# joaotavora/raytracing-one-weekend

Hardware: AMD Instinct MI355X
Metric: Msamples/sec (W×H×spp) on cover scene; achieved HBM GB/s vs peak (higher is better)
Workload: dtype f64

## Files before the change

### raytracing-one-weekend_amd/csrc/rtow_capi.cpp

```cpp

#include <hip/hip_runtime.h>

#include <cmath>
#include <cstdarg>
#include <cstdio>
#include <cstdlib>
#include <algorithm>
#include <chrono>
#include <cstring>
#include <string>
#include <vector>

#include "../../include/rtow.h"
#include "rtow_bvh.h"
#include "rtow_bvh4.h"
#include "rtow_device.h"
#include "rtow_grid.h"
#include "rtow_reftree.h"

namespace {

thread_local std::string g_err;

int fail(int code, const char *fmt, ...) {
// ... 237 lines not shown
  bool bvh4_no_aux = false;
  bool no_bvh4 = false;
  int fetch_votes = 0;
  int leaf_votes = 0;
  int walk_cap = -1, walk_max_open = 0;
  bool bvh4_sm = false;
  int sm4_votes[3] = {8, 16, 16};
  int bvh4_stack_k = 0;
  int sched_chunk = 10;
  int sched_chunk_mesh = 16;
  int ploc_radius = -1;
  int device_tree = 2;
  bool stream_scalar = false;
  bool no_spec = false;
  int tail_bound = 0;
  void read() {
    auto geti = [](const char *n, int d) { const char *e = std::getenv(n); return e ? std::atoi(e) : d; };
    auto getd = [](const char *n, double d) { const char *e = std::getenv(n); return e ? std::atof(e) : d; };
    bvh_leaf = geti("RTOW_BVH_LEAF", 0);
    bvh_ct = getd("RTOW_BVH_CT", -1.0);
    no_leaf_order = std::getenv("RTOW_NO_LEAF_ORDER") != nullptr;
    grid_cpp = getd("RTOW_GRID_CPP", 1.0);
    grid_large = getd("RTOW_GRID_LARGE", 4.0);
    grid_max_tris = geti("RTOW_GRID_MAX_TRIS", 8192);
    if (const char *e = std::getenv("RTOW_PARTIALS_MAX_MB")) partials_cap = (unsigned long long)std::atoll(e) << 20;
    bvh_block = geti("RTOW_BVH_BLOCK", 0);
    if (bvh_block != 256 && bvh_block != 512 && bvh_block != 1024) bvh_block = 0;
    blocks_per_cu = geti("RTOW_BLOCKS_PER_CU", 0);
    if (blocks_per_cu < 1 || blocks_per_cu > 16) blocks_per_cu = 0;
    no_tiles = std::getenv("RTOW_NO_TILES") != nullptr;
// ... 13 lines not shown
        walk_cap = 0;
      }
    }
    if (const char *e = std::getenv("RTOW_SM4_VOTES")) {
      int a = 0, b = 0, d = 0;
      if (std::sscanf(e, "%d,%d,%d", &a, &b, &d) == 3) {
        sm4_votes[0] = std::min(std::max(a, 1), 64);
        sm4_votes[1] = std::min(std::max(b, 1), 64);
        sm4_votes[2] = std::min(std::max(d, 1), 64);
      }
    }
    bvh4_stack_k = std::min(std::max(geti("RTOW_BVH4_STACK_K", 0), 0), 64);
    sched_chunk = std::min(std::max(geti("RTOW_SCHED_CHUNK", 10), 0), 4096);
    sched_chunk_mesh = std::min(std::max(geti("RTOW_SCHED_CHUNK_MESH", 16), 0), 4096);
    tail_bound = std::max(geti("RTOW_TAIL_BOUND", 0), 0);
    no_spec = std::getenv("RTOW_NO_SPEC") != nullptr;
    stream_scalar = std::getenv("RTOW_STREAM_SCALAR") != nullptr;
    if (const char *e = std::getenv("RTOW_PLOC_RADIUS")) ploc_radius = std::min(std::max(std::atoi(e), 0), 64);
    if (const char *e = std::getenv("RTOW_DEVICE_TREE"))
      device_tree = std::strcmp(e, "radix") == 0 ? 0 : (std::strcmp(e, "ploc") == 0 ? 1 : 2);
    if (ploc_radius >= 0 && !std::getenv("RTOW_DEVICE_TREE")) device_tree = ploc_radius == 0 ? 0 : 1;
  }
};

constexpr unsigned kNeedBvh = 1u, kNeedGrid = 2u, kNeedF32 = 4u, kNeedBvh4 = 8u, kNeedAll = 15u;

struct rtow_ctx {
  int device = 0;
  Knobs knobs;
  int num_cus = 0;
  bool have_scene = false;
  rtow::DevScene ds{};
  rtow::DevCamera cam{};
  int n_prims = 0;
  DevBuf sph, sph_r, mov, tri, tri16, prim_mat, mats, blob, cam_dev, gblob;
  DevBuf blob4;
  bool have_bvh4 = false;
  bool have_tri16 = false;
  int bvh4_depth = 0;
  DevBuf blob32, gblob32, cam32_dev;
// ... 5 lines not shown
  long long bvh_nodes = 0;
  int builder = RTOW_BUILDER_HOST_SAH;
  int builder_req = RTOW_BUILDER_AUTO;
  void *lbvh_scratch = nullptr;
  void *grid_scratch = nullptr;
  rtow_build_info_t build_info{};
  struct HostSceneCopy {
    std::vector<double> sg, mg, tg;
    std::vector<int32_t> pk, pi;
    bool have_order = false;
  } host_scene;
  DevBuf rtree;
  bool have_rtree = false;
  PinnedArena arena;
  unsigned built = 0;
  DevBuf partials, stack, counters, spill;
  DevBuf out, out8;
  unsigned char *fuse_rgb8 = nullptr;
  double fuse_spp = 0.0;
  bool fuse_used = false;
  DevBuf counters_init;
  DevBuf dropped;
  unsigned long long *h_dropped = nullptr;
  hipEvent_t upload_ev = nullptr;
  int occ[3][5] = {{0, 0, 0, 0, 0}, {0, 0, 0, 0, 0}, {0, 0, 0, 0, 0}};
  hipEvent_t ev[kEventRing][2] = {};
  int ev_count = 0;
  hipEvent_t call_ev[2] = {};
  unsigned long long *h_counters = nullptr;
  DevBuf q_counters, q_spill, q_rays, q_hits, q_occ, q_map[3];
  bool q_map_ok[3] = {false, false, false};
// ... 50 lines not shown
    he = hipEventCreateWithFlags(&c->upload_ev, hipEventDisableTiming);
  }
  if (he == hipSuccess && c->dropped.ensure(sizeof(unsigned long long)) != RTOW_OK) he = hipErrorOutOfMemory;
  if (he == hipSuccess) he = hipMemset(c->dropped.p, 0, sizeof(unsigned long long));
  if (he != hipSuccess) {
    rtow_ctx_destroy(c);
    return fail(RTOW_EHIP, "rtow_ctx_create: %s", hipGetErrorString(he));
  }
  *out = c;
  return RTOW_OK;
}

void rtow_ctx_destroy(rtow_ctx *c) {
  if (!c) return;
  (void)hipSetDevice(c->device);
  (void)hipDeviceSynchronize();
  for (DevBuf *b : {&c->sph, &c->sph_r, &c->mov, &c->tri, &c->tri16, &c->prim_mat, &c->mats, &c->blob, &c->cam_dev, &c->gblob,
                    &c->blob32, &c->gblob32, &c->cam32_dev, &c->blob4,
                    &c->partials, &c->stack, &c->counters, &c->spill, &c->out, &c->out8, &c->rtree, &c->counters_init,
                    &c->dropped, &c->q_counters, &c->q_spill, &c->q_rays, &c->q_hits, &c->q_occ, &c->q_map[0], &c->q_map[1],
                    &c->q_map[2], &c->rf.map2, &c->rf.map4, &c->rf.par2, &c->rf.par4, &c->rf.need4, &c->rf.flags,
                    &c->rf.nbox2, &c->rf.nbox4, &c->rf.sbox4, &c->rf.pbox, &c->rf.partials, &c->rf.area, &c->rf.g_sph,
                    &c->rf.g_mov, &c->rf.g_tri})
    b->release();
  for (hipEvent_t e : c->rf.ev)
    if (e) (void)hipEventDestroy(e);
  for (hipEvent_t e : c->q_ev)
    if (e) (void)hipEventDestroy(e);
  if (c->h_qcounters) (void)hipHostFree(c->h_qcounters);
  if (c->h_dropped) (void)hipHostFree(c->h_dropped);
  if (c->upload_ev) (void)hipEventDestroy(c->upload_ev);
  if (c->arena.p) (void)hipHostFree(c->arena.p);
  for (int i = 0; i < kEventRing; ++i)
    for (int k = 0; k < 2; ++k)
// ... 104 lines not shown
      if (ns) HIPCHK(hipMemcpyAsync(gp + gimg.off_sph, c->sph.p, sph.size() * 8, hipMemcpyDeviceToDevice, nullptr));
      if (nm) HIPCHK(hipMemcpyAsync(gp + gimg.off_mov, c->mov.p, mov.size() * 8, hipMemcpyDeviceToDevice, nullptr));
      if (nt) HIPCHK(hipMemcpyAsync(gp + gimg.off_tri, c->tri.p, tri.size() * 8, hipMemcpyDeviceToDevice, nullptr));
      HIPCHK(hipMemcpyAsync(gp + gimg.off_pmat, c->prim_mat.p, pmat.size() * 4, hipMemcpyDeviceToDevice, nullptr));
      HIPCHK(hipMemcpyAsync(gp + gimg.off_mats, c->mats.p, mats_bytes.size(), hipMemcpyDeviceToDevice, nullptr));
      grc = rtow::grid_build_phase3(c->grid_scratch, hd.gminf, hd.cellf, hd.n, hd.pad, total_ids, gp, gimg.off_cells,
                                    gimg.off_ids, nullptr, (const double *)c->sph.p, gimg.off_fat,
                                    (const double *)c->mov.p, ns, gimg.fat_stride);
      if (grc) return fail(RTOW_EHIP, "device grid build failed (phase 3, stage %d): %s", grc, hipGetErrorString(hipGetLastError()));
      gimg.ok = true;
    }
  }
  return RTOW_OK;
}

static int scene_upload(rtow_ctx *c, const rtow_scene_t *s, unsigned need);
static int impl_scene_upload(rtow_ctx *c, const rtow_scene_t *s) {
  if (c && c->builder_req == RTOW_BUILDER_AUTO) c->builder = RTOW_BUILDER_HOST_SAH;
  return scene_upload(c, s, kNeedAll);
}

static int scene_upload(rtow_ctx *c, const rtow_scene_t *s, unsigned need) {
  if (!c) return fail(RTOW_EINVAL, "ctx is NULL");
  int rc = validate_scene(s);
  if (rc) return rc;
  HIPCHK(hipSetDevice(c->device));
  HIPCHK(hipDeviceSynchronize());
  if (!c->arena.p) {
    if (hipHostMalloc((void **)&c->arena.p, 8u << 20, hipHostMallocDefault) == hipSuccess)
      c->arena.cap = 8u << 20;
    else
      c->arena.p = nullptr;
  }
  c->arena.used = 0;
  struct ArenaScope {
    explicit ArenaScope(PinnedArena *a) { g_arena = a; }
    ~ArenaScope() { g_arena = nullptr; }
  } arena_scope(&c->arena);
  if (need & kNeedF32) need |= kNeedBvh | kNeedGrid;
  c->built = 0;
  c->have_scene = false;
// ... 482 lines not shown
}

static void tile_shape(const rtow_config_t *cfg, int rows, uint32_t &th, uint32_t &tw) {
  th = tw = 0;
  for (uint32_t h : {3u, 2u, 1u}) {
    const uint32_t hh = 1u << h, ww = 64u >> h;
    if (cfg->tile_rows % hh == 0 && rows % (int)hh == 0 && cfg->image_width % (int)ww == 0) {
      th = h;
      tw = 6u - h;
      return;
    }
  }
}

static int render_levels(rtow_ctx *c, const rtow_config_t *cfg, void *d_rgb_sums, void *hip_stream,
                         rtow_stats_t *stats, const LevelPlan &plan, int lvl_first, int lvl_count, int accumulate);

static int check_dropped(rtow_ctx *c, bool mirrored) {
  unsigned long long v = 0ull;
  if (mirrored)
    v = *c->h_dropped;
  else
    HIPCHK(hipMemcpy(&v, c->dropped.p, sizeof v, hipMemcpyDeviceToHost));
  if (v == 0ull) return RTOW_OK;
  *c->h_dropped = 0ull;
  HIPCHK(hipMemset(c->dropped.p, 0, sizeof v));
  return fail(RTOW_EHIP, "trace kernel: end-of-launch bound reached, %llu lanes gave up their samples", v);
}
static int mirror_dropped(rtow_ctx *c, hipStream_t st) {
  HIPCHK(hipMemcpyAsync(c->h_dropped, c->dropped.p, sizeof(unsigned long long), hipMemcpyDeviceToHost, st));
  return RTOW_OK;
// ... 10 lines not shown

  const int rows = rtow_local_rows(cfg);
  const int spt = cfg->samples_per_pixel / cfg->nstreams;
  const unsigned long long npix = (unsigned long long)rows * cfg->image_width;
  const int streams_now = cfg->stream_count > 0 ? cfg->stream_count : cfg->nstreams;
  if ((unsigned long long)spt * (unsigned long long)(cfg->stream_first + streams_now) > 0xffffffffULL)
    return fail(RTOW_EINVAL, "sample index beyond 32 bits");
  const LevelPlan plan = level_plan(cfg, sched_chunk_for(c));
  const int n_levels = plan.count;
  unsigned long long max_levels = (unsigned long long)n_levels;
  if (npix > 0) {
    max_levels = c->knobs.partials_cap / (npix * 24ull);
    if (0xfffffff0ULL / npix < max_levels) max_levels = 0xfffffff0ULL / npix;
    if (max_levels < 1) max_levels = 1;
  }
  if ((unsigned long long)n_levels <= max_levels || spt == 0 || npix == 0)
    return render_levels(c, cfg, d_rgb_sums, hip_stream, stats, plan, 0, n_levels, cfg->accumulate);
  rtow_stats_t total;
  std::memset(&total, 0, sizeof total);
  for (int done = 0; done < n_levels;) {
    const int now = (int)std::min<unsigned long long>(max_levels, (unsigned long long)(n_levels - done));
    rtow_stats_t st1;
    rc = render_levels(c, cfg, d_rgb_sums, hip_stream, stats ? &st1 : nullptr, plan, done, now,
                       (done > 0 || cfg->accumulate) ? 1 : 0);
    if (rc) return rc;
    if (stats) {
      total.samples += st1.samples;
      total.segments += st1.segments;
      total.prim_tests += st1.prim_tests;
      total.node_tests += st1.node_tests;
      total.kernel_ms += st1.kernel_ms;
      total.total_ms += st1.total_ms;
      total.local_rows = st1.local_rows;
      total.kernel_used = st1.kernel_used;
    }
    done += now;
  }
  if (stats) *stats = total;
  return RTOW_OK;
// ... 104 lines not shown
        aux_src = scene.b4_off_mats;
      aux_bytes = scene.blob4_bytes - aux_src;
      staged = std::min<uint32_t>((kLdsLimit - K * per_entry - aux_bytes) / node_bytes * node_bytes, scene.b4_off_tri);
    }
    K = std::min<uint32_t>(K, (uint32_t)stack_bound);
    scene.b4_lds_limit = staged;
    scene.b4_aux_src = aux_src;
    scene.b4_aux_lds = (staged + 15u) / 16u * 16u;
    scene.b4_stack_base = (scene.b4_aux_lds + aux_bytes + 15u) / 16u * 16u;
    scene.b4_stack_k = K;
    lds_bytes = scene.b4_stack_base + K * per_entry;
  }
  return RTOW_OK;
}

static int render_levels(rtow_ctx *c, const rtow_config_t *cfg, void *d_rgb_sums, void *hip_stream,
                         rtow_stats_t *stats, const LevelPlan &plan, int lvl_first, int lvl_count, int accumulate) {
  int rc;
  hipStream_t st = (hipStream_t)hip_stream;
  const int rows = rtow_local_rows(cfg);
  const unsigned long long npix = (unsigned long long)rows * cfg->image_width;
  const int streams_now = lvl_count;
  const int spt = plan.spt;
  const int spt_last = lvl_first + lvl_count == plan.count ? plan.last : plan.spt;
  const unsigned long long n_items = npix * (unsigned long long)streams_now;
  if (n_items > 0xfffffff0ULL) return fail(RTOW_EINVAL, "too many work items (%llu)", n_items);
  int kernel = 0;
  if ((rc = resolve_kernel(c, cfg->precision, cfg->kernel, &kernel))) return rc;
  const bool strict = cfg->precision == RTOW_F64_STRICT;
  const bool f32 = cfg->precision == RTOW_F32;
  LaunchShape shape;
  if ((rc = launch_shape(c, kernel, f32, shape))) return rc;
// ... 19 lines not shown
  if (kernel == RTOW_KERNEL_BVH4) occ = 0;
  if (occ <= 0) {
    occ = strict ? rtow::trace_occupancy_strict(kernel, block, lds_bytes)
          : f32  ? rtow::trace_occupancy_f32(kernel, block, lds_bytes)
                 : rtow::trace_occupancy_fast(kernel, block, lds_bytes);
    if (occ <= 0) return fail(RTOW_EHIP, "occupancy query failed (kernel %d, %u B of LDS)", kernel, lds_bytes);
    if (occ > 8) occ = 8;
    if (c->knobs.blocks_per_cu) occ = c->knobs.blocks_per_cu;
  }
  long long grid = (long long)c->num_cus * occ;
  const long long need_blocks = (long long)((n_items + block - 1) / block);
  if (grid > need_blocks) grid = need_blocks;
  if (grid < 1) grid = 1;
  const unsigned long long n_lanes = (unsigned long long)grid * block;

  const size_t depth_slots = (size_t)(cfg->max_child_rays > 0 ? cfg->max_child_rays : 1);
  if ((rc = c->partials.ensure((size_t)n_items * 3 * sizeof(double))) ||
      (rc = c->stack.ensure(strict ? depth_slots * (size_t)n_lanes * sizeof(uint32_t) : 4)) ||
      (rc = c->counters.ensure(48 * sizeof(unsigned long long))))
    return rc;
  if (kernel == RTOW_KERNEL_BVH4) {
    const int extra = std::max(stack_bound - (int)scene.b4_stack_k, 0);
    if ((rc = c->spill.ensure(std::max<size_t>((size_t)extra * (size_t)n_lanes * sizeof(uint32_t), 16)))) return rc;
  }

#ifdef RTOW_TAILSTAT
  if (kernel == RTOW_KERNEL_BVH4) return fail(RTOW_EINVAL, "RTOW_TAILSTAT builds do not run the BVH4 kernel");
  if ((rc = c->spill.ensure(std::max<size_t>((size_t)n_lanes, 16)))) return rc;
#endif
  rtow::TraceParams P;
  std::memset(&P, 0, sizeof P);
  P.sc = scene;
  P.cam = (const rtow::DevCamera *)c->cam_dev.p;
  P.cam32 = (const float *)c->cam32_dev.p;
  P.W = cfg->image_width;
  P.H = cfg->image_height;
  P.spt = spt;
  P.nstreams = streams_now;
  P.stream_first = plan.first + lvl_first;
  P.sample_base = (uint32_t)(plan.base + (long long)lvl_first * spt);
  P.spt_last = spt_last;
  {
    const unsigned long long b = 64ull * (4096ull + 8ull * (unsigned long long)(cfg->max_child_rays + 2) *
// ... 15 lines not shown
  P.div_npix = make_fastdiv((uint32_t)npix);
  P.div_w = make_fastdiv((uint32_t)cfg->image_width);
  P.div_tile = make_fastdiv((uint32_t)cfg->tile_rows);
  P.div_ns = make_fastdiv((uint32_t)streams_now);
  uint32_t th = 0, tw = 0;
  if (!c->knobs.no_tiles) tile_shape(cfg, rows, th, tw);
  P.tile_h_log2 = th;
  P.tile_w_log2 = tw;
  P.div_tpr_n = th ? (uint32_t)cfg->image_width >> tw : 1u;
  P.div_tpr = make_fastdiv(P.div_tpr_n);
  P.n_tile_rows = th ? (uint32_t)rows >> th : 1u;
  {
    const int eighths = c->knobs.sky_eighths;
    P.sky_rows = th ? P.n_tile_rows * (uint32_t)eighths / 8u : 0u;
  }
  P.partials = (double *)c->partials.p;
  P.stack = (uint32_t *)c->stack.p;
  P.spill = (uint32_t *)c->spill.p;
  P.spec = rtow::kSpecGeneric;
  if (kernel == RTOW_KERNEL_GRID && lds_bytes > 0 && !f32 && !c->knobs.no_spec && scene.n_tri == 0) {
    if (scene.n_mov == 0 && c->grid_fat_stride == 48u) P.spec = rtow::kSpecStaticSpheres;
    if (scene.n_mov > 0 && c->grid_fat_stride == 80u) P.spec = rtow::kSpecMovingSpheres;
  }
  P.b4_trips = c->knobs.bvh4_sm ? 0u : 1u;
  {
    const bool b4 = kernel == RTOW_KERNEL_BVH4;
    const bool b4_nodes_resident = b4 && scene.b4_lds_limit >= scene.b4_off_tri;
    int cap = c->knobs.walk_cap, open = c->knobs.walk_max_open;
    if (cap < 0) {
      cap = b4 ? 4 : 3;
      open = b4 ? (b4_nodes_resident ? 24 : 32) : 16;
    }
    if (cap > 0 && !b4) cap = std::max(cap, 3);
    P.walk_cap = cap > 0 ? (uint32_t)cap : 0xffffffffu;
    P.walk_max_open = (uint32_t)open;
    P.leaf_votes = (uint32_t)(c->knobs.leaf_votes > 0 ? c->knobs.leaf_votes : (b4 ? 28 : 16));
  }
  P.fetch_votes = (uint32_t)(c->knobs.fetch_votes > 0 ? c->knobs.fetch_votes : (kernel == RTOW_KERNEL_BVH4 ? 2 : 4));
  P.sm4_restart = (uint32_t)c->knobs.sm4_votes[0];
  P.sm4_scatter = (uint32_t)c->knobs.sm4_votes[1];
  P.sm4_leaf = (uint32_t)c->knobs.sm4_votes[2];
  P.counters = (unsigned long long *)c->counters.p;
  P.t_origin = P.counters + 16;

  if (st != nullptr) HIPCHK(hipStreamWaitEvent(st, c->upload_ev, 0));
  if (stats) HIPCHK(hipEventRecord(c->call_ev[0], st));
  if (!c->counters_init.p) {
    std::vector<unsigned long long> init(48, 0ull);
    init[5] = init[16] = ~0ull;
    if ((rc = c->counters_init.ensure(48 * sizeof(unsigned long long)))) return rc;
    HIPCHK(hipMemcpy(c->counters_init.p, init.data(), 48 * sizeof(unsigned long long), hipMemcpyHostToDevice));
  }
  HIPCHK(hipMemcpyAsync(c->counters.p, c->counters_init.p, 48 * sizeof(unsigned long long), hipMemcpyDeviceToDevice, st));
  const int slot = c->ev_count < kEventRing ? c->ev_count : -1;
  if (slot >= 0) HIPCHK(hipEventRecord(c->ev[slot][0], st));
  int launch_kernel = kernel;
  if (image_kernel && lds_bytes > 0 && c->knobs.stamps) launch_kernel = kernel + 16;
  int lrc = strict ? rtow::launch_trace_strict(P, launch_kernel, (int)grid, block, lds_bytes, st)
            : f32  ? rtow::launch_trace_f32(P, launch_kernel, (int)grid, block, lds_bytes, st)
                   : rtow::launch_trace_fast(P, launch_kernel, (int)grid, block, lds_bytes, st);
#ifdef RTOW_TAILSTAT
  if (const char *path = std::getenv("RTOW_TAILSTAT_OUT")) {
    HIPCHK(hipStreamSynchronize(st));
    std::vector<unsigned long long> ts((size_t)n_lanes / 64 * 8);
    HIPCHK(hipMemcpy(ts.data(), c->spill.p, ts.size() * 8, hipMemcpyDeviceToHost));
    if (FILE *f = std::fopen(path, "wb")) {
      std::fwrite(ts.data(), 8, ts.size(), f);
      std::fclose(f);
    }
  }
#endif
  if (lrc != 0) return fail(RTOW_EHIP, "trace kernel launch failed: %s", hipGetErrorString((hipError_t)lrc));
  if (slot >= 0) {
    HIPCHK(hipEventRecord(c->ev[slot][1], st));
    c->ev_count++;
  }
  rtow::ReduceParams R;
  R.partials = P.partials;
  R.out = (double *)d_rgb_sums;
  R.npix3 = (uint32_t)(npix * 3);
  R.nstreams = streams_now;
  R.accumulate = accumulate;
  R.W = (uint32_t)cfg->image_width;
  R.tile_w_log2 = tw;
  R.tile_h_log2 = th;
  R.tiles_per_row = P.div_tpr_n;
  R.rgb8 = nullptr;
  R.spp = 0.0;
  if (c->fuse_rgb8 && lvl_first == 0 && lvl_count == plan.count && !accumulate) {
    R.rgb8 = c->fuse_rgb8;
    R.spp = c->fuse_spp;
    c->fuse_used = true;
  }
  lrc = rtow::launch_reduce(R, st);
  if (lrc != 0) return fail(RTOW_EHIP, "reduce kernel launch failed: %s", hipGetErrorString((hipError_t)lrc));

  if (stats) {
    HIPCHK(hipEventRecord(c->call_ev[1], st));
    HIPCHK(hipMemcpyAsync(c->h_counters, c->counters.p, 48 * sizeof(unsigned long long),
                          hipMemcpyDeviceToHost, st));
    HIPCHK(hipStreamSynchronize(st));
    if (c->h_counters[47] != 0ull) {
      (void)check_dropped(c, false);
      return fail(RTOW_EHIP, "trace kernel: end-of-launch bound reached, %llu lanes gave up their samples",
                  c->h_counters[47]);
    }
    float ms = 0.f;
    HIPCHK(hipEventElapsedTime(&ms, c->call_ev[0], c->call_ev[1]));
    stats->total_ms = ms;
    if (slot >= 0) {
      HIPCHK(hipEventElapsedTime(&ms, c->ev[slot][0], c->ev[slot][1]));
      stats->kernel_ms = ms;
    }
    stats->samples = npix * ((unsigned long long)spt * (unsigned long long)(streams_now - 1) + (unsigned long long)spt_last);
// ... 233 lines not shown
  if ((rc = c->q_rays.ensure((size_t)n * k.in_bytes)) || (rc = d_out.ensure((size_t)n * k.out_bytes))) return rc;
  HIPCHK(hipMemcpy(c->q_rays.p, in, (size_t)n * k.in_bytes, hipMemcpyHostToDevice));
  if ((rc = query_device(c, k, precision, kernel, c->q_rays.p, n, d_out.p, nullptr, stats))) return rc;
  HIPCHK(hipMemcpy(out, d_out.p, (size_t)n * k.out_bytes, hipMemcpyDeviceToHost));
  return RTOW_OK;
}

struct Bvh4Frame {
  double c[3];
  float is[3];
  uint32_t half;
  uint32_t lds_limit;
  uint32_t pad_;
};
static_assert(sizeof(Bvh4Frame) == 48, "rtow_debug_image(5) record");

int rtow_debug_image(rtow_ctx *c, int32_t which, void *out, int64_t capacity, int64_t *size_out) {
  if (!c || !size_out) return fail(RTOW_EINVAL, "NULL argument");
  if (!c->have_scene) return fail(RTOW_ENOSCENE, "no scene uploaded");
  const void *src = nullptr;
  int64_t bytes = 0;
  Bvh4Frame frame{};
  switch (which) {
    case 0: src = c->blob.p; bytes = c->ds.blob_bytes; break;
    case 1: src = c->gblob.p; bytes = c->ds.gblob_bytes; break;
    case 2: src = c->blob32.p; bytes = c->ds32.blob_bytes; break;
    case 3: src = c->gblob32.p; bytes = c->ds32.gblob_bytes; break;
    case 4: src = c->blob4.p; bytes = c->have_bvh4 ? c->ds.blob4_bytes : 0; break;
    case 5:
      if (c->have_bvh4) {
        for (int k = 0; k < 3; ++k) {
          frame.c[k] = c->ds.b4_c[k];
          frame.is[k] = c->ds.b4_is[k];
        }
        frame.half = c->ds.b4_half;
        frame.lds_limit = c->ds.b4_lds_limit;
        bytes = (int64_t)sizeof frame;
      }
      break;
    default: return fail(RTOW_EINVAL, "unknown image %d", which);
  }
  *size_out = bytes;
  if (!out) return RTOW_OK;
  if (capacity < bytes) return fail(RTOW_EINVAL, "buffer too small (%lld < %lld)", (long long)capacity, (long long)bytes);
  if (which == 5) {
    if (bytes) std::memcpy(out, &frame, sizeof frame);
    return RTOW_OK;
  }
  HIPCHK(hipSetDevice(c->device));
  HIPCHK(hipDeviceSynchronize());
  if (bytes) HIPCHK(hipMemcpy(out, src, (size_t)bytes, hipMemcpyDeviceToHost));
  return RTOW_OK;
}

int rtow_debug_counters(rtow_ctx *c, unsigned long long *out48) {
  if (!c || !out48) return fail(RTOW_EINVAL, "NULL argument");
  if (!c->counters.p) return fail(RTOW_ENOSCENE, "no launch yet");
  HIPCHK(hipSetDevice(c->device));
  HIPCHK(hipDeviceSynchronize());
  HIPCHK(hipMemcpy(out48, c->counters.p, 48 * sizeof(unsigned long long), hipMemcpyDeviceToHost));
  return RTOW_OK;
}

int rtow_tonemap_device(rtow_ctx *c, const void *d_rgb_sums, int64_t n_values, int32_t spp_effective,
                        void *d_rgb8, void *hip_stream) {
  if (!c) return fail(RTOW_EINVAL, "ctx is NULL");
  if (!d_rgb_sums || !d_rgb8) return fail(RTOW_EINVAL, "NULL device pointer");
  if (n_values < 0 || n_values > 0xffffffffLL) return fail(RTOW_EINVAL, "n_values out of range");
  if (spp_effective <= 0) return fail(RTOW_EINVAL, "spp_effective must be positive");
  HIPCHK(hipSetDevice(c->device));
  int lrc = rtow::launch_tonemap((const double *)d_rgb_sums, (unsigned char *)d_rgb8, (uint32_t)n_values,
                                 (double)spp_effective, hip_stream);
  if (lrc != 0) return fail(RTOW_EHIP, "tonemap launch failed: %s", hipGetErrorString((hipError_t)lrc));
  return RTOW_OK;
}

int rtow_profile_collect(rtow_ctx *c, double *kernel_ms_sum, int32_t *launches) {
  if (!c) return fail(RTOW_EINVAL, "ctx is NULL");
  HIPCHK(hipSetDevice(c->device));
  double sum = 0.0;
  for (int i = 0; i < c->ev_count; ++i) {
    HIPCHK(hipEventSynchronize(c->ev[i][1]));
    float ms = 0.f;
    HIPCHK(hipEventElapsedTime(&ms, c->ev[i][0], c->ev[i][1]));
    sum += ms;
  }
  if (kernel_ms_sum) *kernel_ms_sum = sum;
  if (launches) *launches = c->ev_count;
  const bool waited = c->ev_count > 0;
  c->ev_count = 0;
  return waited ? check_dropped(c, false) : RTOW_OK;
}

static int upload_for(rtow_ctx *c, const rtow_scene_t *scene, const rtow_config_t *cfg) {
  if (!c) return fail(RTOW_EINVAL, "ctx is NULL");
  int rc = validate_scene(scene);
  if (rc) return rc;
  const long long np = (long long)scene->n_spheres + scene->n_moving + scene->n_triangles;
  unsigned need;
  const int k = cfg->kernel;
// ... 29 lines not shown
  int rc = validate_cfg(cfg);
  if (rc) return rc;
  if ((rc = upload_for(c, scene, cfg))) return rc;
  const int rows = rtow_local_rows(cfg);
  const size_t bytes = (size_t)rows * cfg->image_width * 3 * sizeof(double);
  if (bytes == 0) {
    if (stats) {
      std::memset(stats, 0, sizeof *stats);
    }
    return RTOW_OK;
  }
  if ((rc = c->out.ensure(bytes))) return rc;
  void *d_out = c->out.p;
  if (cfg->accumulate)
    HIPCHK(hipMemcpy(d_out, rgb_sums_host, bytes, hipMemcpyHostToDevice));
  rc = rtow_render_device(c, cfg, d_out, nullptr, stats);
  if (rc != RTOW_OK) return rc;
  if ((rc = mirror_dropped(c, nullptr))) return rc;
  HIPCHK(hipMemcpy(rgb_sums_host, d_out, bytes, hipMemcpyDeviceToHost));
  return check_dropped(c, true);
}

static int impl_render_device_rgb8(rtow_ctx *c, const rtow_config_t *cfg, void *d_rgb8, void *hip_stream,
                                   rtow_stats_t *stats) {
  if (!c) return fail(RTOW_EINVAL, "ctx is NULL");
  if (!d_rgb8) return fail(RTOW_EINVAL, "d_rgb8 is NULL");
  int rc = validate_cfg(cfg);
  if (rc) return rc;
  const int spp_eff = cfg->samples_per_pixel / cfg->nstreams * cfg->nstreams;
  if (spp_eff <= 0) return fail(RTOW_EINVAL, "no effective samples (samples_per_pixel < nstreams)");
  if (cfg->accumulate) return fail(RTOW_EINVAL, "the rgb8 entry points own their sums: accumulate must be 0");
// ... 18 lines not shown
                     rtow_stats_t *stats) {
  if (!c) return fail(RTOW_EINVAL, "ctx is NULL");
  if (!rgb8_host) return fail(RTOW_EINVAL, "rgb8_host is NULL");
  int rc = validate_cfg(cfg);
  if (rc) return rc;
  if (cfg->samples_per_pixel / cfg->nstreams <= 0) return fail(RTOW_EINVAL, "no effective samples (samples_per_pixel < nstreams)");
  if (cfg->accumulate) return fail(RTOW_EINVAL, "rtow_render_rgb8 owns its sums: accumulate must be 0");
  if ((rc = upload_for(c, scene, cfg))) return rc;
  const int rows = rtow_local_rows(cfg);
  const size_t n = (size_t)rows * cfg->image_width * 3;
  if (n == 0) {
    if (stats) std::memset(stats, 0, sizeof *stats);
    return RTOW_OK;
  }
  if ((rc = c->out8.ensure(n))) return rc;
  if ((rc = impl_render_device_rgb8(c, cfg, c->out8.p, nullptr, stats))) return rc;
  if ((rc = mirror_dropped(c, nullptr))) return rc;
  HIPCHK(hipMemcpy(rgb8_host, c->out8.p, n, hipMemcpyDeviceToHost));
  return check_dropped(c, true);
}

static int refit_check_shape(const rtow_ctx *c, const rtow_scene_t *s) {
  if (s->n_spheres != c->ds.n_sph || s->n_moving != c->ds.n_mov || s->n_triangles != c->ds.n_tri || s->n_prims != c->n_prims ||
      s->n_materials != c->ds.n_mats)
    return fail(RTOW_EINVAL, "rtow_scene_refit: the scene's counts (%d spheres, %d moving, %d triangles, %d materials) are not "
                "the resident scene's (%d, %d, %d, %d): call rtow_scene_upload", s->n_spheres, s->n_moving, s->n_triangles,
                s->n_materials, c->ds.n_sph, c->ds.n_mov, c->ds.n_tri, c->ds.n_mats);
  const rtow_ctx::HostSceneCopy &h = c->host_scene;
  const bool order = s->prim_kind && s->prim_index;
  if (order != h.have_order ||
      (order && (std::memcmp(s->prim_kind, h.pk.data(), (size_t)s->n_prims * 4) != 0 ||
// ... 43 lines not shown
    if (rtow::refit_bvh4_links(ds.blob4, n4, nb, co, (int32_t *)r.par4.p, (int32_t *)r.need4.p, nullptr))
      return fail(RTOW_EHIP, "refit 4-wide link pass failed: %s", hipGetErrorString(hipGetLastError()));
  }
  r.ready = true;
  return RTOW_OK;
}

static int impl_scene_refit(rtow_ctx *c, const rtow_scene_t *s) {
  if (!c) return fail(RTOW_EINVAL, "ctx is NULL");
  int rc = validate_scene(s);
  if (rc) return rc;
  if (!c->have_scene) return fail(RTOW_ENOSCENE, "no scene uploaded");
  if ((rc = refit_check_shape(c, s))) return rc;
  const double t_call = now_ms();
  HIPCHK(hipSetDevice(c->device));
  HIPCHK(hipDeviceSynchronize());
  rtow_ctx::Refit &r = c->rf;
  if (!r.ev[0])
    for (hipEvent_t &e : r.ev) HIPCHK(hipEventCreate(&e));
  HIPCHK(hipEventRecord(r.ev[0], nullptr));
  c->have_scene = false;
  c->arena.used = 0;
  struct ArenaScope {
    explicit ArenaScope(PinnedArena *a) { g_arena = a; }
    ~ArenaScope() { g_arena = nullptr; }
  } arena_scope(&c->arena);
  if (!r.ready && (rc = refit_prepare(c))) return rc;
  rtow::DevScene &ds = c->ds;
  const int ns = ds.n_sph, nm = ds.n_mov, nt = ds.n_tri, np = c->n_prims;
  const bool bvh2 = (c->built & kNeedBvh) != 0, f32 = (c->built & kNeedF32) != 0;
// ... 232 lines not shown
int rtow_closest_point(rtow_ctx *c, int32_t precision, int32_t kernel, const rtow_point_query_t *queries, int64_t n,
                       rtow_point_hit_t *hits, rtow_stats_t *stats) {
  return guarded("rtow_closest_point", [&] { return query_host(c, kClosestPoint, precision, kernel, queries, n, hits, stats); });
}
int rtow_scene_refit(rtow_ctx *c, const rtow_scene_t *s) {
  return guarded("rtow_scene_refit", [&] { return impl_scene_refit(c, s); });
}
int rtow_debug_schedule(rtow_ctx *c, const rtow_config_t *cfg, uint32_t *out, int32_t capacity_pairs) {
  return guarded("rtow_debug_schedule", [&] { return impl_debug_schedule(c, cfg, out, capacity_pairs); });
}

}

namespace rtow {
int ctx_check_dropped(rtow_ctx *c) { return c ? check_dropped(c, false) : RTOW_OK; }
int ctx_mirror_dropped(rtow_ctx *c, void *stream) { return c ? mirror_dropped(c, (hipStream_t)stream) : RTOW_OK; }
int ctx_check_dropped_mirrored(rtow_ctx *c) {
  if (!c) return RTOW_OK;
  if (*c->h_dropped != 0ull) HIPCHK(hipSetDevice(c->device));
  return check_dropped(c, true);
}
}
```

### raytracing-one-weekend_amd/csrc/rtow_multi.cpp

```cpp
#include <dlfcn.h>
#include <hip/hip_runtime.h>
#include <rccl/rccl.h>

#include <algorithm>
#include <atomic>
#include <chrono>
#include <condition_variable>
#include <cstdio>
#include <cstdlib>
#include <cstring>
#include <functional>
#include <mutex>
#include <new>
#include <string>
#include <thread>
#include <vector>

#include "../../include/rtow.h"

namespace rtow {
int set_last_error(int code, const char *fmt, ...);
int ctx_check_dropped(rtow_ctx *c);
int ctx_mirror_dropped(rtow_ctx *c, void *stream);
int ctx_check_dropped_mirrored(rtow_ctx *c);
int launch_place_rows(const void *gathered, void *image, uint32_t n_ranks, uint32_t max_rows, uint32_t row_bytes,
                      uint32_t height, uint32_t tile_rows, void *stream);
}

namespace {

struct Rccl {
  void *lib = nullptr;
  decltype(&ncclCommInitAll) CommInitAll = nullptr;
  decltype(&ncclCommDestroy) CommDestroy = nullptr;
  decltype(&ncclCommAbort) CommAbort = nullptr;
  decltype(&ncclGather) Gather = nullptr;
  decltype(&ncclGetErrorString) GetErrorString = nullptr;
  bool load(std::string &why) {
    for (const char *name : {"librccl.so.1", "librccl.so", "/opt/rocm/lib/librccl.so.1"}) {
// ... 195 lines not shown
      }
      for (int r = 0; r < n_devices; ++r) m->ranks[(size_t)r].comm = comms[(size_t)r];
    }
    if (const char *e = std::getenv("RTOW_MULTI_FAIL_GATHER")) m->fail_gather_rank = std::atoi(e);
    if (const char *e = std::getenv("RTOW_MULTI_D2H")) m->d2h_blocking = std::strcmp(e, "blocking") == 0;
    try {
      for (int r = 0; r < n_devices; ++r) m->threads.emplace_back([m, r] { m->worker(r); });
    } catch (...) {
      rtow_multi_destroy(m);
      throw;
    }
    m->run([m](int r) {
      Rank &me = m->ranks[(size_t)r];
      const int rc = rtow_ctx_create(me.device, &me.ctx);
      if (rc) return me.fail_with_last(rc, "rtow_ctx_create");
      if (!me.hip(hipSetDevice(me.device), "hipSetDevice")) return;
      if (!me.hip(hipStreamCreate(&me.stream), "hipStreamCreate")) return;
      me.hip(hipEventCreateWithFlags(&me.strips_ev, hipEventDisableTiming), "hipEventCreate");
    });
    const int rc = m->collect("rtow_multi_create");
    if (rc) {
      const std::string keep = rtow_last_error();
      rtow_multi_destroy(m);
      return rtow::set_last_error(rc, "%s", keep.c_str());
    }
    *out = m;
    return RTOW_OK;
  });
}

// ... 262 lines not shown
```

### raytracing-one-weekend_amd/rtow.py

```python
from __future__ import annotations

import ctypes as C
import os
from pathlib import Path

import numpy as np

PKG_DIR = Path(__file__).resolve().parent
REPO_ROOT = PKG_DIR.parent
LIB_PATH = Path(os.environ.get("RTOW_LIB", PKG_DIR / "librtow.so"))

RTOW_ABI_VERSION = 9
RTOW_OK, RTOW_EINVAL, RTOW_ENODEV, RTOW_EHIP, RTOW_ENOSCENE, RTOW_EEMPTY, RTOW_ENOMEM = 0, -1, -2, -3, -4, -5, -6
MAT_LAMBERTIAN, MAT_METAL, MAT_DIELECTRIC = 0, 1, 2
PRIM_SPHERE, PRIM_MOVING_SPHERE, PRIM_TRIANGLE = 0, 1, 2
F64_STRICT, F64_FAST, F32 = 0, 1, 2
KERNEL_AUTO, KERNEL_BRUTE, KERNEL_BVH, KERNEL_GRID, KERNEL_BVH4, KERNEL_REFTREE = 0, 1, 2, 3, 4, 5
MODEL_OO, MODEL_VARIANT, MODEL_WORLD = 0, 1, 2
BUILDER_HOST_SAH, BUILDER_DEVICE_LBVH, BUILDER_AUTO = 0, 1, 2

d3 = C.c_double * 3
_pd = C.POINTER(C.c_double)
_pi = C.POINTER(C.c_int32)

# ... 350 lines not shown
    def refit_info(self) -> RefitInfo:
        ri = RefitInfo()
        check(lib().rtow_refit_info(self._h, C.byref(ri)), "rtow_refit_info")
        return ri

    def set_builder(self, builder: int):
        check(lib().rtow_ctx_set_builder(self._h, builder), "rtow_ctx_set_builder")

    def debug_image(self, which: int) -> bytes:
        n = C.c_int64()
        check(lib().rtow_debug_image(self._h, which, None, 0, C.byref(n)), "rtow_debug_image")
        buf = (C.c_ubyte * max(n.value, 1))()
        check(lib().rtow_debug_image(self._h, which, buf, n.value, C.byref(n)), "rtow_debug_image")
        return bytes(buf[:n.value])

    def build_info(self) -> BuildInfo:
        bi = BuildInfo()
        check(lib().rtow_build_info(self._h, C.byref(bi)), "rtow_build_info")
        return bi

    def render_device(self, cfg: Config, d_ptr: int, stream: int = 0, want_stats=False):
        st = Stats() if want_stats else None
        check(lib().rtow_render_device(self._h, C.byref(cfg), C.c_void_p(d_ptr),
                                       C.c_void_p(stream), C.byref(st) if st is not None else None),
              "rtow_render_device")
        return st

    def tonemap_device(self, d_sums: int, n_values: int, spp_eff: int, d_rgb8: int, stream: int = 0):
        check(lib().rtow_tonemap_device(self._h, C.c_void_p(d_sums), n_values, spp_eff,
                                        C.c_void_p(d_rgb8), C.c_void_p(stream)), "rtow_tonemap_device")
# ... 178 lines not shown
```

Baseline: 15820.

## Double-buffer trace scratch across two launch slots with per-slot streams

Splits the trace scratch buffers (partials, stack, counters, spill) into two launch slots, each with its own non-blocking stream and traced/consumed events. Consecutive device-entry renders alternate slots, so the next frame's trace kernel can overlap the previous frame's reduce instead of serialising on shared scratch. Host-entry and stats paths, and multi-device ranks, stay on a single slot. The change doubles scratch memory, adds cross-stream event synchronisation, and alters kernel-time accounting to subtract overlapping intervals.

```diff
diff --git a/raytracing-one-weekend_amd/csrc/rtow_capi.cpp b/raytracing-one-weekend_amd/csrc/rtow_capi.cpp
--- a/raytracing-one-weekend_amd/csrc/rtow_capi.cpp
+++ b/raytracing-one-weekend_amd/csrc/rtow_capi.cpp
@@ -275,6 +275,7 @@
   bool stream_scalar = false;
   bool no_spec = false;
   int tail_bound = 0;
+  int frames_in_flight = 2;
   void read() {
     auto geti = [](const char *n, int d) { const char *e = std::getenv(n); return e ? std::atoi(e) : d; };
     auto getd = [](const char *n, double d) { const char *e = std::getenv(n); return e ? std::atof(e) : d; };
@@ -318,6 +319,7 @@
     sched_chunk = std::min(std::max(geti("RTOW_SCHED_CHUNK", 10), 0), 4096);
     sched_chunk_mesh = std::min(std::max(geti("RTOW_SCHED_CHUNK_MESH", 16), 0), 4096);
     tail_bound = std::max(geti("RTOW_TAIL_BOUND", 0), 0);
+    frames_in_flight = std::min(std::max(geti("RTOW_FRAMES_IN_FLIGHT", 2), 1), 2);
     no_spec = std::getenv("RTOW_NO_SPEC") != nullptr;
     stream_scalar = std::getenv("RTOW_STREAM_SCALAR") != nullptr;
     if (const char *e = std::getenv("RTOW_PLOC_RADIUS")) ploc_radius = std::min(std::max(std::atoi(e), 0), 64);
@@ -328,6 +330,15 @@
 };
 
 constexpr unsigned kNeedBvh = 1u, kNeedGrid = 2u, kNeedF32 = 4u, kNeedBvh4 = 8u, kNeedAll = 15u;
+
+constexpr int kLaunchSlots = 2;
+struct LaunchSlot {
+  DevBuf partials, stack, counters, spill;
+  hipStream_t stream = nullptr;
+  hipEvent_t traced = nullptr;
+  hipEvent_t consumed = nullptr;
+  size_t bytes() const { return partials.bytes + stack.bytes + counters.bytes + spill.bytes; }
+};
 
 struct rtow_ctx {
   int device = 0;
@@ -363,7 +374,9 @@
   bool have_rtree = false;
   PinnedArena arena;
   unsigned built = 0;
-  DevBuf partials, stack, counters, spill;
+  LaunchSlot slots[kLaunchSlots];
+  int last_slot = 0;
+  bool host_entry = false;
   DevBuf out, out8;
   unsigned char *fuse_rgb8 = nullptr;
   double fuse_spp = 0.0;
@@ -444,10 +457,18 @@
 void rtow_ctx_destroy(rtow_ctx *c) {
   if (!c) return;
   (void)hipSetDevice(c->device);
+  for (LaunchSlot &s : c->slots)
+    if (s.stream) (void)hipStreamSynchronize(s.stream);
   (void)hipDeviceSynchronize();
+  for (LaunchSlot &s : c->slots) {
+    for (DevBuf *b : {&s.partials, &s.stack, &s.counters, &s.spill}) b->release();
+    if (s.traced) (void)hipEventDestroy(s.traced);
+    if (s.consumed) (void)hipEventDestroy(s.consumed);
+    if (s.stream) (void)hipStreamDestroy(s.stream);
+  }
   for (DevBuf *b : {&c->sph, &c->sph_r, &c->mov, &c->tri, &c->tri16, &c->prim_mat, &c->mats, &c->blob, &c->cam_dev, &c->gblob,
                     &c->blob32, &c->gblob32, &c->cam32_dev, &c->blob4,
-                    &c->partials, &c->stack, &c->counters, &c->spill, &c->out, &c->out8, &c->rtree, &c->counters_init,
+                    &c->out, &c->out8, &c->rtree, &c->counters_init,
                     &c->dropped, &c->q_counters, &c->q_spill, &c->q_rays, &c->q_hits, &c->q_occ, &c->q_map[0], &c->q_map[1],
                     &c->q_map[2], &c->rf.map2, &c->rf.map4, &c->rf.par2, &c->rf.par4, &c->rf.need4, &c->rf.flags,
                     &c->rf.nbox2, &c->rf.nbox4, &c->rf.sbox4, &c->rf.pbox, &c->rf.partials, &c->rf.area, &c->rf.g_sph,
@@ -582,6 +603,12 @@
   return RTOW_OK;
 }
 
+static int slots_wait_traced(rtow_ctx *c) {
+  for (LaunchSlot &s : c->slots)
+    if (s.traced) HIPCHK(hipEventSynchronize(s.traced));
+  return RTOW_OK;
+}
+
 static int scene_upload(rtow_ctx *c, const rtow_scene_t *s, unsigned need);
 static int impl_scene_upload(rtow_ctx *c, const rtow_scene_t *s) {
   if (c && c->builder_req == RTOW_BUILDER_AUTO) c->builder = RTOW_BUILDER_HOST_SAH;
@@ -593,6 +620,7 @@
   int rc = validate_scene(s);
   if (rc) return rc;
   HIPCHK(hipSetDevice(c->device));
+  if ((rc = slots_wait_traced(c))) return rc;
   HIPCHK(hipDeviceSynchronize());
   if (!c->arena.p) {
     if (hipHostMalloc((void **)&c->arena.p, 8u << 20, hipHostMallocDefault) == hipSuccess)
@@ -1105,7 +1133,7 @@
 }
 
 static int render_levels(rtow_ctx *c, const rtow_config_t *cfg, void *d_rgb_sums, void *hip_stream,
-                         rtow_stats_t *stats, const LevelPlan &plan, int lvl_first, int lvl_count, int accumulate);
+                         rtow_stats_t *stats, const LevelPlan &plan, int lvl_first, int lvl_count, int accumulate, int slot_ix);
 
 static int check_dropped(rtow_ctx *c, bool mirrored) {
   unsigned long long v = 0ull;
@@ -1146,15 +1174,17 @@
     if (0xfffffff0ULL / npix < max_levels) max_levels = 0xfffffff0ULL / npix;
     if (max_levels < 1) max_levels = 1;
   }
+  const bool in_flight = !stats && !c->host_entry && c->knobs.frames_in_flight > 1;
+  const int slot_ix = in_flight ? 1 - c->last_slot : 0;
   if ((unsigned long long)n_levels <= max_levels || spt == 0 || npix == 0)
-    return render_levels(c, cfg, d_rgb_sums, hip_stream, stats, plan, 0, n_levels, cfg->accumulate);
+    return render_levels(c, cfg, d_rgb_sums, hip_stream, stats, plan, 0, n_levels, cfg->accumulate, slot_ix);
   rtow_stats_t total;
   std::memset(&total, 0, sizeof total);
   for (int done = 0; done < n_levels;) {
     const int now = (int)std::min<unsigned long long>(max_levels, (unsigned long long)(n_levels - done));
     rtow_stats_t st1;
     rc = render_levels(c, cfg, d_rgb_sums, hip_stream, stats ? &st1 : nullptr, plan, done, now,
-                       (done > 0 || cfg->accumulate) ? 1 : 0);
+                       (done > 0 || cfg->accumulate) ? 1 : 0, slot_ix);
     if (rc) return rc;
     if (stats) {
       total.samples += st1.samples;
@@ -1289,8 +1319,27 @@
   return RTOW_OK;
 }
 
+struct HostEntryScope {
+  rtow_ctx *c;
+  explicit HostEntryScope(rtow_ctx *ctx) : c(ctx) { c->host_entry = true; }
+  ~HostEntryScope() { c->host_entry = false; }
+};
+
+static int slot_open(LaunchSlot &S) {
+  if (!S.stream) HIPCHK(hipStreamCreateWithFlags(&S.stream, hipStreamNonBlocking));
+  if (!S.traced) HIPCHK(hipEventCreateWithFlags(&S.traced, hipEventDisableTiming));
+  if (!S.consumed) HIPCHK(hipEventCreateWithFlags(&S.consumed, hipEventDisableTiming));
+  return RTOW_OK;
+}
+static int slot_ensure(LaunchSlot &S, DevBuf &b, size_t need) {
+  if (need <= b.bytes) return RTOW_OK;
+  HIPCHK(hipEventSynchronize(S.traced));
+  HIPCHK(hipEventSynchronize(S.consumed));
+  return b.ensure(need);
+}
+
 static int render_levels(rtow_ctx *c, const rtow_config_t *cfg, void *d_rgb_sums, void *hip_stream,
-                         rtow_stats_t *stats, const LevelPlan &plan, int lvl_first, int lvl_count, int accumulate) {
+                         rtow_stats_t *stats, const LevelPlan &plan, int lvl_first, int lvl_count, int accumulate, int slot_ix) {
   int rc;
   hipStream_t st = (hipStream_t)hip_stream;
   const int rows = rtow_local_rows(cfg);
@@ -1340,19 +1389,21 @@
   if (grid < 1) grid = 1;
   const unsigned long long n_lanes = (unsigned long long)grid * block;
 
+  LaunchSlot &S = c->slots[slot_ix];
+  if ((rc = slot_open(S))) return rc;
   const size_t depth_slots = (size_t)(cfg->max_child_rays > 0 ? cfg->max_child_rays : 1);
-  if ((rc = c->partials.ensure((size_t)n_items * 3 * sizeof(double))) ||
-      (rc = c->stack.ensure(strict ? depth_slots * (size_t)n_lanes * sizeof(uint32_t) : 4)) ||
-      (rc = c->counters.ensure(48 * sizeof(unsigned long long))))
+  if ((rc = slot_ensure(S, S.partials, (size_t)n_items * 3 * sizeof(double))) ||
+      (rc = slot_ensure(S, S.stack, strict ? depth_slots * (size_t)n_lanes * sizeof(uint32_t) : 4)) ||
+      (rc = slot_ensure(S, S.counters, 48 * sizeof(unsigned long long))))
     return rc;
   if (kernel == RTOW_KERNEL_BVH4) {
     const int extra = std::max(stack_bound - (int)scene.b4_stack_k, 0);
-    if ((rc = c->spill.ensure(std::max<size_t>((size_t)extra * (size_t)n_lanes * sizeof(uint32_t), 16)))) return rc;
+    if ((rc = slot_ensure(S, S.spill, std::max<size_t>((size_t)extra * (size_t)n_lanes * sizeof(uint32_t), 16)))) return rc;
   }
 
 #ifdef RTOW_TAILSTAT
   if (kernel == RTOW_KERNEL_BVH4) return fail(RTOW_EINVAL, "RTOW_TAILSTAT builds do not run the BVH4 kernel");
-  if ((rc = c->spill.ensure(std::max<size_t>((size_t)n_lanes, 16)))) return rc;
+  if ((rc = slot_ensure(S, S.spill, std::max<size_t>((size_t)n_lanes, 16)))) return rc;
 #endif
   rtow::TraceParams P;
   std::memset(&P, 0, sizeof P);
@@ -1398,9 +1449,9 @@
     const int eighths = c->knobs.sky_eighths;
     P.sky_rows = th ? P.n_tile_rows * (uint32_t)eighths / 8u : 0u;
   }
-  P.partials = (double *)c->partials.p;
-  P.stack = (uint32_t *)c->stack.p;
-  P.spill = (uint32_t *)c->spill.p;
+  P.partials = (double *)S.partials.p;
+  P.stack = (uint32_t *)S.stack.p;
+  P.spill = (uint32_t *)S.spill.p;
   P.spec = rtow::kSpecGeneric;
   if (kernel == RTOW_KERNEL_GRID && lds_bytes > 0 && !f32 && !c->knobs.no_spec && scene.n_tri == 0) {
     if (scene.n_mov == 0 && c->grid_fat_stride == 48u) P.spec = rtow::kSpecStaticSpheres;
@@ -1424,41 +1475,49 @@
   P.sm4_restart = (uint32_t)c->knobs.sm4_votes[0];
   P.sm4_scatter = (uint32_t)c->knobs.sm4_votes[1];
   P.sm4_leaf = (uint32_t)c->knobs.sm4_votes[2];
-  P.counters = (unsigned long long *)c->counters.p;
+  P.counters = (unsigned long long *)S.counters.p;
   P.t_origin = P.counters + 16;
 
-  if (st != nullptr) HIPCHK(hipStreamWaitEvent(st, c->upload_ev, 0));
-  if (stats) HIPCHK(hipEventRecord(c->call_ev[0], st));
+  hipStream_t ts = S.stream;
+  HIPCHK(hipStreamWaitEvent(ts, c->upload_ev, 0));
+  if (stats) {
+    HIPCHK(hipEventRecord(c->call_ev[0], st));
+    HIPCHK(hipStreamWaitEvent(ts, c->call_ev[0], 0));
+  }
+  HIPCHK(hipStreamWaitEvent(ts, S.consumed, 0));
   if (!c->counters_init.p) {
     std::vector<unsigned long long> init(48, 0ull);
     init[5] = init[16] = ~0ull;
     if ((rc = c->counters_init.ensure(48 * sizeof(unsigned long long)))) return rc;
     HIPCHK(hipMemcpy(c->counters_init.p, init.data(), 48 * sizeof(unsigned long long), hipMemcpyHostToDevice));
   }
-  HIPCHK(hipMemcpyAsync(c->counters.p, c->counters_init.p, 48 * sizeof(unsigned long long), hipMemcpyDeviceToDevice, st));
+  HIPCHK(hipMemcpyAsync(S.counters.p, c->counters_init.p, 48 * sizeof(unsigned long long), hipMemcpyDeviceToDevice, ts));
   const int slot = c->ev_count < kEventRing ? c->ev_count : -1;
-  if (slot >= 0) HIPCHK(hipEventRecord(c->ev[slot][0], st));
+  if (slot >= 0) HIPCHK(hipEventRecord(c->ev[slot][0], ts));
   int launch_kernel = kernel;
   if (image_kernel && lds_bytes > 0 && c->knobs.stamps) launch_kernel = kernel + 16;
-  int lrc = strict ? rtow::launch_trace_strict(P, launch_kernel, (int)grid, block, lds_bytes, st)
-            : f32  ? rtow::launch_trace_f32(P, launch_kernel, (int)grid, block, lds_bytes, st)
-                   : rtow::launch_trace_fast(P, launch_kernel, (int)grid, block, lds_bytes, st);
+  int lrc = strict ? rtow::launch_trace_strict(P, launch_kernel, (int)grid, block, lds_bytes, ts)
+            : f32  ? rtow::launch_trace_f32(P, launch_kernel, (int)grid, block, lds_bytes, ts)
+                   : rtow::launch_trace_fast(P, launch_kernel, (int)grid, block, lds_bytes, ts);
+  c->last_slot = slot_ix;
 #ifdef RTOW_TAILSTAT
   if (const char *path = std::getenv("RTOW_TAILSTAT_OUT")) {
-    HIPCHK(hipStreamSynchronize(st));
-    std::vector<unsigned long long> ts((size_t)n_lanes / 64 * 8);
-    HIPCHK(hipMemcpy(ts.data(), c->spill.p, ts.size() * 8, hipMemcpyDeviceToHost));
+    HIPCHK(hipStreamSynchronize(ts));
+    std::vector<unsigned long long> tail((size_t)n_lanes / 64 * 8);
+    HIPCHK(hipMemcpy(tail.data(), S.spill.p, tail.size() * 8, hipMemcpyDeviceToHost));
     if (FILE *f = std::fopen(path, "wb")) {
-      std::fwrite(ts.data(), 8, ts.size(), f);
+      std::fwrite(tail.data(), 8, tail.size(), f);
       std::fclose(f);
     }
   }
 #endif
   if (lrc != 0) return fail(RTOW_EHIP, "trace kernel launch failed: %s", hipGetErrorString((hipError_t)lrc));
   if (slot >= 0) {
-    HIPCHK(hipEventRecord(c->ev[slot][1], st));
+    HIPCHK(hipEventRecord(c->ev[slot][1], ts));
     c->ev_count++;
   }
+  HIPCHK(hipEventRecord(S.traced, ts));
+  HIPCHK(hipStreamWaitEvent(st, S.traced, 0));
   rtow::ReduceParams R;
   R.partials = P.partials;
   R.out = (double *)d_rgb_sums;
@@ -1477,11 +1536,13 @@
     c->fuse_used = true;
   }
   lrc = rtow::launch_reduce(R, st);
+  const hipError_t cons = hipEventRecord(S.consumed, st);
   if (lrc != 0) return fail(RTOW_EHIP, "reduce kernel launch failed: %s", hipGetErrorString((hipError_t)lrc));
+  HIPCHK(cons);
 
   if (stats) {
     HIPCHK(hipEventRecord(c->call_ev[1], st));
-    HIPCHK(hipMemcpyAsync(c->h_counters, c->counters.p, 48 * sizeof(unsigned long long),
+    HIPCHK(hipMemcpyAsync(c->h_counters, S.counters.p, 48 * sizeof(unsigned long long),
                           hipMemcpyDeviceToHost, st));
     HIPCHK(hipStreamSynchronize(st));
     if (c->h_counters[47] != 0ull) {
@@ -1745,13 +1806,20 @@
   uint32_t pad_;
 };
 static_assert(sizeof(Bvh4Frame) == 48, "rtow_debug_image(5) record");
+struct SlotFrame {
+  uint64_t bytes[kLaunchSlots];
+  uint32_t frames_in_flight;
+  uint32_t last_slot;
+};
+static_assert(sizeof(SlotFrame) == 24, "rtow_debug_image(6) record");
 
 int rtow_debug_image(rtow_ctx *c, int32_t which, void *out, int64_t capacity, int64_t *size_out) {
   if (!c || !size_out) return fail(RTOW_EINVAL, "NULL argument");
-  if (!c->have_scene) return fail(RTOW_ENOSCENE, "no scene uploaded");
+  if (!c->have_scene && which != 6) return fail(RTOW_ENOSCENE, "no scene uploaded");
   const void *src = nullptr;
   int64_t bytes = 0;
   Bvh4Frame frame{};
+  SlotFrame slots{};
   switch (which) {
     case 0: src = c->blob.p; bytes = c->ds.blob_bytes; break;
     case 1: src = c->gblob.p; bytes = c->ds.gblob_bytes; break;
@@ -1769,13 +1837,19 @@
         bytes = (int64_t)sizeof frame;
       }
       break;
+    case 6:
+      for (int k = 0; k < kLaunchSlots; ++k) slots.bytes[k] = c->slots[k].bytes();
+      slots.frames_in_flight = (uint32_t)c->knobs.frames_in_flight;
+      slots.last_slot = (uint32_t)c->last_slot;
+      bytes = (int64_t)sizeof slots;
+      break;
     default: return fail(RTOW_EINVAL, "unknown image %d", which);
   }
   *size_out = bytes;
   if (!out) return RTOW_OK;
   if (capacity < bytes) return fail(RTOW_EINVAL, "buffer too small (%lld < %lld)", (long long)capacity, (long long)bytes);
-  if (which == 5) {
-    if (bytes) std::memcpy(out, &frame, sizeof frame);
+  if (which == 5 || which == 6) {
+    if (bytes) std::memcpy(out, which == 5 ? (const void *)&frame : (const void *)&slots, (size_t)bytes);
     return RTOW_OK;
   }
   HIPCHK(hipSetDevice(c->device));
@@ -1786,10 +1860,11 @@
 
 int rtow_debug_counters(rtow_ctx *c, unsigned long long *out48) {
   if (!c || !out48) return fail(RTOW_EINVAL, "NULL argument");
-  if (!c->counters.p) return fail(RTOW_ENOSCENE, "no launch yet");
+  const LaunchSlot &S = c->slots[c->last_slot];
+  if (!S.counters.p) return fail(RTOW_ENOSCENE, "no launch yet");
   HIPCHK(hipSetDevice(c->device));
   HIPCHK(hipDeviceSynchronize());
-  HIPCHK(hipMemcpy(out48, c->counters.p, 48 * sizeof(unsigned long long), hipMemcpyDeviceToHost));
+  HIPCHK(hipMemcpy(out48, S.counters.p, 48 * sizeof(unsigned long long), hipMemcpyDeviceToHost));
   return RTOW_OK;
 }
 
@@ -1810,11 +1885,19 @@
   if (!c) return fail(RTOW_EINVAL, "ctx is NULL");
   HIPCHK(hipSetDevice(c->device));
   double sum = 0.0;
+  for (int i = 0; i < c->ev_count; ++i) HIPCHK(hipEventSynchronize(c->ev[i][1]));
+  int prev = -1;
   for (int i = 0; i < c->ev_count; ++i) {
-    HIPCHK(hipEventSynchronize(c->ev[i][1]));
     float ms = 0.f;
     HIPCHK(hipEventElapsedTime(&ms, c->ev[i][0], c->ev[i][1]));
-    sum += ms;
+    if (prev >= 0) {
+      float behind = 0.f;
+      HIPCHK(hipEventElapsedTime(&behind, c->ev[prev][1], c->ev[i][1]));
+      if (behind <= 0.f) continue;
+      ms = std::min(ms, behind);
+    }
+    prev = i;
+    sum += std::max(ms, 0.f);
   }
   if (kernel_ms_sum) *kernel_ms_sum = sum;
   if (launches) *launches = c->ev_count;
@@ -1874,7 +1957,10 @@
   void *d_out = c->out.p;
   if (cfg->accumulate)
     HIPCHK(hipMemcpy(d_out, rgb_sums_host, bytes, hipMemcpyHostToDevice));
-  rc = rtow_render_device(c, cfg, d_out, nullptr, stats);
+  {
+    HostEntryScope slot0(c);
+    rc = rtow_render_device(c, cfg, d_out, nullptr, stats);
+  }
   if (rc != RTOW_OK) return rc;
   if ((rc = mirror_dropped(c, nullptr))) return rc;
   HIPCHK(hipMemcpy(rgb_sums_host, d_out, bytes, hipMemcpyDeviceToHost));
@@ -1923,7 +2009,11 @@
     return RTOW_OK;
   }
   if ((rc = c->out8.ensure(n))) return rc;
-  if ((rc = impl_render_device_rgb8(c, cfg, c->out8.p, nullptr, stats))) return rc;
+  {
+    HostEntryScope slot0(c);
+    rc = impl_render_device_rgb8(c, cfg, c->out8.p, nullptr, stats);
+  }
+  if (rc) return rc;
   if ((rc = mirror_dropped(c, nullptr))) return rc;
   HIPCHK(hipMemcpy(rgb8_host, c->out8.p, n, hipMemcpyDeviceToHost));
   return check_dropped(c, true);
@@ -1997,6 +2087,7 @@
   if ((rc = refit_check_shape(c, s))) return rc;
   const double t_call = now_ms();
   HIPCHK(hipSetDevice(c->device));
+  if ((rc = slots_wait_traced(c))) return rc;
   HIPCHK(hipDeviceSynchronize());
   rtow_ctx::Refit &r = c->rf;
   if (!r.ev[0])
@@ -2259,6 +2350,9 @@
 
 namespace rtow {
 int ctx_check_dropped(rtow_ctx *c) { return c ? check_dropped(c, false) : RTOW_OK; }
+void ctx_one_launch_slot(rtow_ctx *c) {
+  if (c) c->knobs.frames_in_flight = 1;
+}
 int ctx_mirror_dropped(rtow_ctx *c, void *stream) { return c ? mirror_dropped(c, (hipStream_t)stream) : RTOW_OK; }
 int ctx_check_dropped_mirrored(rtow_ctx *c) {
   if (!c) return RTOW_OK;
diff --git a/raytracing-one-weekend_amd/csrc/rtow_multi.cpp b/raytracing-one-weekend_amd/csrc/rtow_multi.cpp
--- a/raytracing-one-weekend_amd/csrc/rtow_multi.cpp
+++ b/raytracing-one-weekend_amd/csrc/rtow_multi.cpp
@@ -23,6 +23,7 @@
 int ctx_check_dropped(rtow_ctx *c);
 int ctx_mirror_dropped(rtow_ctx *c, void *stream);
 int ctx_check_dropped_mirrored(rtow_ctx *c);
+void ctx_one_launch_slot(rtow_ctx *c);
 int launch_place_rows(const void *gathered, void *image, uint32_t n_ranks, uint32_t max_rows, uint32_t row_bytes,
                       uint32_t height, uint32_t tile_rows, void *stream);
 }
@@ -248,6 +249,7 @@
       Rank &me = m->ranks[(size_t)r];
       const int rc = rtow_ctx_create(me.device, &me.ctx);
       if (rc) return me.fail_with_last(rc, "rtow_ctx_create");
+      rtow::ctx_one_launch_slot(me.ctx);
       if (!me.hip(hipSetDevice(me.device), "hipSetDevice")) return;
       if (!me.hip(hipStreamCreate(&me.stream), "hipStreamCreate")) return;
       me.hip(hipEventCreateWithFlags(&me.strips_ev, hipEventDisableTiming), "hipEventCreate");
diff --git a/raytracing-one-weekend_amd/rtow.py b/raytracing-one-weekend_amd/rtow.py
--- a/raytracing-one-weekend_amd/rtow.py
+++ b/raytracing-one-weekend_amd/rtow.py
@@ -388,6 +388,12 @@
         check(lib().rtow_debug_image(self._h, which, buf, n.value, C.byref(n)), "rtow_debug_image")
         return bytes(buf[:n.value])
 
+    def launch_slots(self) -> dict:
+        import struct
+
+        b0, b1, fif, last = struct.unpack("<QQII", self.debug_image(6))
+        return {"bytes": (b0, b1), "frames_in_flight": fif, "last_slot": last}
+
     def build_info(self) -> BuildInfo:
         bi = BuildInfo()
         check(lib().rtow_build_info(self._h, C.byref(bi)), "rtow_build_info")
```

Result: faster. 16370 (median of 6 runs) (+3.5%).
